# sarpaykent/GotenNet

Measured on AMD Instinct MI355X. Metric: molecules/sec (energy+force forward), rMD17 aspirin batch=128, 1/2/4/8 MI355X, higher is better.
Workload: dtype f32 (2xfp16-split MFMA with block exponents, fp32 accumulate); 1 GPU; rmd17_aspirin batch=128/GPU (N=2688 atoms, E=54368 edges incl. self-loops), n_atom_basis=256, n_interactions=6, lmax=2, n_rbf=32, heads=8, sep_dir/sep_tensor, energy+forces; global_batch=128, parallelism=dp1 (molecule shards, 1 all-reduce)

## Files before the change

gotennet_amd/_lib.py:

```python
from __future__ import annotations

import ctypes as C
import os

_PKG = os.path.dirname(os.path.abspath(__file__))
LIB_PATH = os.environ.get("GN_LIB_PATH") or os.path.join(_PKG, "libgotennet_hip.so")

GN_ERR_BAD_ARG = 10001
ABI_VERSION = 11
LMAX_SLICED = 0x100
LMAX_MEAN, LMAX_MAX = 0x200, 0x400

ACT_NONE = 11
WGRAD_F32, WGRAD_F16X2 = 0, 2
_P, _I, _F, _L, _D = C.c_void_p, C.c_int, C.c_float, C.c_long, C.c_double

class GemmDesc(C.Structure):
    _fields_ = [("A", _P), ("lda", _I), ("W", _P), ("bias", _P), ("C", _P), ("ldc", _I),
                ("M", _I), ("N", _I), ("K", _I), ("act_lo", _I), ("act_hi", _I),
                ("row_cnt", _I), ("row_gstride", _I), ("row_goff", _I),
                ("res", _P), ("gate", _P), ("gate_mode", _I), ("pre_out", _P),
                ("pro_mode", _I), ("pro_lo", _I), ("pro_hi", _I), ("a_pre", _P), ("ldp", _I),
                ("a_gate", _P), ("ldg", _I), ("A2", _P), ("A3", _P), ("a_seg", _I), ("act_kind", _I), ("lda2", _I)]


class WgradDesc(C.Structure):
    _fields_ = [("dY", _P), ("ldy", _I), ("y_off", _I), ("A", _P), ("lda", _I), ("a_off", _I),
                ("dW", _P), ("ldw", _I), ("db", _P), ("rows", _I), ("nout", _I), ("K", _I),
                ("row_cnt", _I), ("row_gstride", _I), ("row_goff", _I)]
# ... 26 lines not shown
    "gn_eqff_fused_backward": [_P, _P, _P, _P, _P, _P, _P, _P, _I, _I, _I, _P, _P, _I, _P],
    "gn_htr_edge": [_P, _P, _P, _P, _P, _I, _I, _I, _I, _P, _P, _P],
    "gn_eqff_context": [_P, _P, _F, _I, _I, _I, _P, _P],
    "gn_eqff_update": [_P, _P, _I, _I, _I, _P, _P, _P],
    "gn_gemm_ex": [_P, _I, _P, _P, _P, _I, _I, _I, _I, _I, _I, _I, _I, _I, _P, _P, _I, _P, _I, _I, _I, _P, _I, _P, _I, _I, _P],
    "gn_gemm_group": [_P, _I, _P],
    "gn_edge_vectors": [_P, _P, _P, _I, _P, _P, _P],
    "gn_gemm_split": [_P, _I, _P, _P, _P, _I, _I, _I, _I, _I, _I, _I, _I, _I, _P, _P, _I, _P, _I, _I, _I, _P, _I, _P, _I, _I, _P],
    "gn_split_bf16x3": [_P, _I, _I, _P, _P],
    "gn_split_bf16x3_size": [_I, _I],
    "gn_gemm_group_split": [_P, _I, _P],
    "gn_gemm_f16x2": [_P, _I, _P, _P, _P, _I, _I, _I, _I, _I, _I, _I, _I, _I, _P, _P, _I, _P, _I, _I, _I, _P, _I, _P, _I, _I, _P],
    "gn_split_f16x2": [_P, _I, _I, _P, _P],
    "gn_split_f16x2_size": [_I, _I],
    "gn_gemm_group_f16x2": [_P, _I, _P],
    "gn_htr_backward": [_P, _P, _P, _P, _P, _P, _P, _P, _P, _P, _P, _P, _I, _I, _I, _I, _P, _P, _P, _P, _I, _P],
    "gn_message_backward": [_P, _P, _I, _P, _I, _P, _P, _I, _P, _P, _P, _P, _P, _P, _P, _P, _P, _P, _P,
                            _P, _P, _P, _I, _P, _P, _P, _P, _P, _P, C.c_long, _I, _I, _I, _I, _I, _I, _I, _P],
    "gn_message_backward_dropout": [_P, _P, _I, _P, _I, _P, _P, _P, _I, _P, _P, _P, _P, _P, _P, _P, _P, _P, _P, _P,
                                    _P, _P, _P, _I, _P, _P, _P, _P, _P, _P, C.c_long, _I, _I, _I, _I, _I, _I, _I, _P],
    "gn_message_backward_groups": [_I, _I, _I, _I],
    "gn_eqff_backward_a": [_P, _P, _P, _P, _I, _I, _I, _P, _P, _P],
    "gn_eqff_backward_b": [_P, _P, _P, _P, _I, _I, _I, _P, _P, _P],
    "gn_edge_init_backward": [_P, _P, _P, _I, _P, _P, _P, _P, _I, _I, _P, _P, _P],
    "gn_node_init_backward": [_P, _P, _P, _I, _P, _P, _P, _P, _I, _I, _P, _P, _P],
    "gn_layernorm_silu_backward": [_P, _P, _P, _F, _P, _I, _I, _P, _I, _P],
    "gn_layernorm_backward": [_P, _P, _F, _P, _I, _I, _P, _P],
    "gn_tensor_norm_backward": [_P, _P, _P, _F, _I, _I, _I, _P, _P],
    "gn_gate": [_P, _I, _L, _P, _P],
    "gn_gate_backward": [_P, _P, _I, _L, _P, _P],
# ... 105 lines not shown
```

gotennet_amd/csrc/gn_gemm.hip:

```cpp
#include <climits>
#include <type_traits>
#include "gn_gemm.h"
#include "gn_tune.h"

namespace gn {

__device__ __forceinline__ float4 keep4(bool ok, const float4& v) {
    return make_float4(ok ? v.x : 0.f, ok ? v.y : 0.f, ok ? v.z : 0.f, ok ? v.w : 0.f);
}
__device__ __forceinline__ float amax4(const float4& v) { return fmaxf(fmaxf(fabsf(v.x), fabsf(v.y)), fmaxf(fabsf(v.z), fabsf(v.w))); }

template <int R>
__device__ __forceinline__ int block_exponent(const float4 (&v)[R]) {
    float m = 0.f;
#pragma unroll
    for (int i = 0; i < R; ++i) m = fmaxf(m, amax4(v[i]));
    int need = (int)((wave_umax_sgpr(__float_as_uint(m)) >> 23) & 0xffu) - 126 - 15;
    if (__builtin_expect(need > 112, 0)) {
        asm volatile("" ::: "memory");
        float mf = 0.f;
#pragma unroll
        for (int i = 0; i < R; ++i) {
            const float c[4] = {v[i].x, v[i].y, v[i].z, v[i].w};
#pragma unroll
            for (int t = 0; t < 4; ++t) mf = fmaxf(mf, fabsf(c[t]) <= 3.0e38f ? fabsf(c[t]) : 0.f);
        }
        need = (int)((wave_umax_sgpr(__float_as_uint(mf)) >> 23) & 0xffu) - 126 - 15;
    }
    return need < -120 ? -120 : need;
}
__device__ __forceinline__ void store_f16x2(_Float16* d, int apl, const float4& v, float scale) {
    f16x4 h, l;
    split4_f16(v, scale, h, l);
    *reinterpret_cast<f16x4*>(d) = h;
    *reinterpret_cast<f16x4*>(d + apl) = l;
}

template <int TM, int TN, int WM, int WN, bool PRO, int MODE, bool ASILU>
__device__ __forceinline__ void gemm_body(const GroupArgs ga) {
    static_assert(WM * WN == 4, "four waves per workgroup");
    constexpr bool SPLIT = MODE != 0;
    constexpr bool F16 = MODE == 2;
    constexpr int NP = F16 ? 2 : 3;
    constexpr int BM = 32 * TM * WM, BN = 32 * TN * WN;
    constexpr int RA = BM / 32, RB = BN / 32;
    constexpr int STAGE = (BM + BN) * PITCH;
    constexpr int CP = BN + 4;
    constexpr int APL = BM * SPLIT_PB;
    constexpr int STAGE_S = NP * APL;
    constexpr int MAIN_FLOATS = SPLIT ? (2 * STAGE_S) / 2 : 2 * STAGE;
    constexpr int LDS_FLOATS = (MAIN_FLOATS > BM * CP) ? MAIN_FLOATS : BM * CP;
    __shared__ __attribute__((aligned(16))) float smem[LDS_FLOATS + (F16 ? 2 : 0)];
    signed char* const exps = reinterpret_cast<signed char*>(smem + LDS_FLOATS);
    int e_run = -120;
    unsigned e_acc = 0x88888888u;
    int ewt = 0;

    int cum[GN_MAX_GROUP], shift[GN_MAX_GROUP];
    const int xcd = blockIdx.x & 7;
    if (ga.spread) {
        int run = 0, prev_end = 0;
#pragma unroll
        for (int gi = 0; gi < GN_MAX_GROUP; ++gi) {
            const int tg = gi < ga.n ? ga.tile_end[gi] - prev_end : 0;
            prev_end = gi < ga.n ? ga.tile_end[gi] : prev_end;
            const XcdCut c = xcd_cut(tg, xcd);
            shift[gi] = c.lo - run;
            run += c.cnt;
            cum[gi] = run;
        }
// ... 32 lines not shown
    const int wave = tid >> 6;
    const int wm = wave / WN, wn = wave % WN;
    const int c4 = tid & 7;
    const int sr = tid >> 3;
    const int stride = gridDim.x >> 3;

    int prow[RA];
    const float* brow[RB];
    bool aok[RA], bok[RB];
    bool a_full = false;
    auto set_tile = [&](int t_idx) {
        const int m0f = ((t_idx - g_begin) / tiles_n) * BM, n0f = ((t_idx - g_begin) % tiles_n) * BN;
        a_full = m0f + BM <= p.M && (p.K % BK) == 0;
#pragma unroll
        for (int i = 0; i < RA; ++i) {
            const int gm = m0f + sr + 32 * i;
            aok[i] = gm < p.M;
            prow[i] = phys_row(p, aok[i] ? gm : 0);
        }
        if constexpr (!SPLIT) {
#pragma unroll
            for (int i = 0; i < RB; ++i) {
                const int gn = n0f + sr + 32 * i;
                bok[i] = gn < p.N;
                brow[i] = p.W + (size_t)(bok[i] ? gn : 0) * p.K + 4 * c4;
            }
        }
    };

    f32x16 acc[TM][TN];

    float4 pa[RA], pb[RB];
    constexpr bool AHEAD = SPLIT && !PRO;
    float4 qa2[2][RA];
    bool kok2[2] = {true, true};
    auto fetchA = [&](int k0, float4 (&qa)[RA], bool& kflag) {
        const int kraw = k0 + 4 * c4;
        const bool kok = kraw < p.K;
// ... 5 lines not shown
            const bool s2 = k0c >= 2 * p.a_seg, s1 = k0c >= p.a_seg;
            Ab = s2 ? p.A3 : (s1 ? p.A2 : p.A);
            ka = kc - (s2 ? 2 * p.a_seg : (s1 ? p.a_seg : 0));
            ld = p.lda + ((p.lda2 - p.lda) & -(int)s1);
        }
#pragma unroll
        for (int i = 0; i < RA; ++i) qa[i] = ld4(Ab + (size_t)prow[i] * ld + ka);
        kflag = kok;
    };
    auto stash_f16 = [&](int sb, const float4 (&v)[RA]) {
        _Float16* d0 = reinterpret_cast<_Float16*>(smem) + sb * STAGE_S + sr * SPLIT_PB + 4 * c4;
        const int need = block_exponent(v);
        e_run = need > e_run ? need : e_run;
        const float scale = exp_scale(e_run);
#pragma unroll
        for (int i = 0; i < RA; ++i) store_f16x2(d0 + 32 * i * SPLIT_PB, APL, v[i], scale);
        if (lane == 0) exps[sb * 4 + wave] = (signed char)e_run;
    };
    auto stash_bf16 = [&](int sb, const float4 (&v)[RA]) {
        __bf16* d0 = reinterpret_cast<__bf16*>(smem) + sb * STAGE_S + sr * SPLIT_PB + 4 * c4;
#pragma unroll
        for (int i = 0; i < RA; ++i) {
            bf16x4 h, m, l;
            split4_trunc(v[i], h, m, l);
            __bf16* d = d0 + 32 * i * SPLIT_PB;
            *reinterpret_cast<bf16x4*>(d) = h;
            *reinterpret_cast<bf16x4*>(d + APL) = m;
            *reinterpret_cast<bf16x4*>(d + 2 * APL) = l;
        }
    };
    auto stashA = [&](int sb, const float4 (&qa)[RA], bool kflag) {
        if constexpr (F16) {
            if (a_full) {
                stash_f16(sb, qa);
                return;
            }
        }
        float4 v[RA];
#pragma unroll
        for (int i = 0; i < RA; ++i) v[i] = keep4(aok[i] && kflag, qa[i]);
// ... 29 lines not shown
        if constexpr (!SPLIT) {
#pragma unroll
            for (int i = 0; i < RB; ++i) qb[i] = (bok[i] && kok) ? ld4(brow[i] + k0) : zero4();
        }
    };
    auto stash = [&](int sb, const float4 (&qa)[RA], const float4 (&qb)[RB]) {
        if constexpr (AHEAD) {
            stashA(sb, qa2[0], kok2[0]);
        } else if constexpr (F16) {
            stash_f16(sb, qa);
        } else if constexpr (SPLIT) {
            stash_bf16(sb, qa);
        } else {
            float* buf = smem + sb * STAGE;
#pragma unroll
            for (int i = 0; i < RA; ++i) st4(&buf[(sr + 32 * i) * PITCH + 4 * c4], qa[i]);
#pragma unroll
            for (int i = 0; i < RB; ++i) st4(&buf[(BM + sr + 32 * i) * PITCH + 4 * c4], qb[i]);
        }
    };
    const uint4* wfrag = reinterpret_cast<const uint4*>(p.W);
    int ks2 = 0;
    size_t nt_off[TN];
    auto set_btile = [&](int n0b) {
        wfrag = reinterpret_cast<const uint4*>(p.W) + (F16 ? 16 : 0);
        if constexpr (F16) ewt = __builtin_amdgcn_readfirstlane(*reinterpret_cast<const int*>(p.W));
        ks2 = 2 * ((p.K + BK - 1) / BK);
        const int nt_last = (p.N + 31) / 32 - 1;
#pragma unroll
        for (int j = 0; j < TN; ++j) {
            int nt = n0b / 32 + wn * TN + j;
            nt = nt < nt_last ? nt : nt_last;
            nt_off[j] = (size_t)nt * ks2 * (NP * 64) + lane;
        }
    };
    auto load_b = [&](int g, uint4 (&q)[TN][NP]) {
#pragma unroll
        for (int j = 0; j < TN; ++j)
#pragma unroll
            for (int s_ = 0; s_ < NP; ++s_) q[j][s_] = wfrag[nt_off[j] + (size_t)(g * NP + s_) * 64];
    };
    auto rescale = [&](int sb) {
        const unsigned en = (unsigned)__builtin_amdgcn_readfirstlane(*reinterpret_cast<const int*>(exps + sb * 4));
        if (__builtin_expect(en != e_acc, 0)) {
            rescale_rows(&acc[0][0], TM * TN, e_acc, en);
            e_acc = en;
        }
    };

    auto kstep = [&](const __bf16* Ap, int ks, const uint4 (&bw)[TN][NP]) {
        if constexpr (F16) {
            f16x8 a[TM][2];
#pragma unroll
            for (int i = 0; i < TM; ++i)
#pragma unroll
                for (int s_ = 0; s_ < 2; ++s_)
                    a[i][s_] = *reinterpret_cast<const f16x8*>(Ap + s_ * APL + i * 32 * SPLIT_PB + ks * 16);
#pragma unroll
            for (int t = 0; t < 3; ++t)
#pragma unroll
                for (int i = 0; i < TM; ++i)
// ... 9 lines not shown
                for (int s_ = 0; s_ < 3; ++s_)
                    a[i][s_] = *reinterpret_cast<const bf16x8*>(Ap + s_ * APL + i * 32 * SPLIT_PB + ks * 16);
            constexpr int TA[6] = {2, 0, 1, 1, 0, 0};
            constexpr int TB[6] = {0, 2, 1, 0, 1, 0};
#pragma unroll
            for (int t = 0; t < 6; ++t)
#pragma unroll
                for (int i = 0; i < TM; ++i)
#pragma unroll
                    for (int j = 0; j < TN; ++j)
                        acc[i][j] = __builtin_amdgcn_mfma_f32_32x32x16_bf16(
                            a[i][TA[t]], __builtin_bit_cast(bf16x8, bw[j][TB[t]]), acc[i][j], 0, 0, 0);
        }
    };

    auto loop_planes_ahead = [&](int nk, uint4 (&bq)[2][TN][NP]) {
        const __bf16* const Abase = reinterpret_cast<const __bf16*>(smem) + (wm * 32 * TM + (lane & 31)) * SPLIT_PB + (lane >> 5) * 8;
        auto slab = [&](int kt, auto SET, auto LAST) {
            constexpr int set = decltype(SET)::value;
            constexpr bool last = decltype(LAST)::value;
            const __bf16* Ap = Abase + set * STAGE_S;
            load_b(2 * kt + 1, bq[1]);
            if constexpr (!last) fetchA((kt + 2) * BK, qa2[set], kok2[set]);
            __builtin_amdgcn_sched_barrier(0);
            if constexpr (F16) rescale(set);
            kstep(Ap, 0, bq[0]);
            __builtin_amdgcn_sched_barrier(0);
            if constexpr (!last) load_b(2 * kt + 2, bq[0]);
            kstep(Ap, 1, bq[1]);
            __builtin_amdgcn_sched_barrier(0);
            if constexpr (!last) stashA(set ^ 1, qa2[set ^ 1], kok2[set ^ 1]);
            __syncthreads();
        };
        using T0 = std::integral_constant<int, 0>; using T1 = std::integral_constant<int, 1>;
        using No = std::false_type; using Yes = std::true_type;
        fetchA(BK, qa2[1], kok2[1]);
        int kt = 0;
        for (; kt + 2 < nk; kt += 2) {
            slab(kt, T0{}, No{});
            slab(kt + 1, T1{}, No{});
        }
        if (nk - kt == 2) {
            slab(kt, T0{}, No{});
            slab(kt + 1, T1{}, Yes{});
        } else {
            slab(kt, T0{}, Yes{});
        }
    };

    int idx = blockIdx.x >> 3;
    if (idx >= tile_stop) return;
    select(idx);
    set_tile(idx);
    fetch(0, pa, pb);
    for (;;) {
        const int nk = (p.K + BK - 1) / BK;
        const int m0 = ((idx - g_begin) / tiles_n) * BM;
        const int n0 = ((idx - g_begin) % tiles_n) * BN;
#pragma unroll
        for (int i = 0; i < TM; ++i)
#pragma unroll
            for (int j = 0; j < TN; ++j)
#pragma unroll
                for (int r = 0; r < 16; ++r) acc[i][j][r] = 0.f;
        if constexpr (F16) {
            e_run = -120;
            e_acc = 0x88888888u;
        }
        stash(0, pa, pb);
        uint4 bq[2][TN][NP];
        if constexpr (SPLIT) {
            set_btile(n0);
            load_b(0, bq[0]);
        }
        __syncthreads();
        if constexpr (AHEAD) loop_planes_ahead(nk, bq);
        else if constexpr (SPLIT) {
            const __bf16* const Abase = reinterpret_cast<const __bf16*>(smem) + (wm * 32 * TM + (lane & 31)) * SPLIT_PB + (lane >> 5) * 8;
            if (nk > 1) fetch(BK, pa, pb);
            for (int kt = 0; kt < nk; ++kt) {
                const __bf16* Ap = Abase + (kt & 1) * STAGE_S;
                load_b(2 * kt + 1, bq[1]);
                if constexpr (F16) rescale(kt & 1);
                kstep(Ap, 0, bq[0]);
                if (kt + 1 < nk) load_b(2 * kt + 2, bq[0]);
                kstep(Ap, 1, bq[1]);
                if (kt + 1 < nk) stash((kt + 1) & 1, pa, pb);
                __syncthreads();
                if (kt + 2 < nk) fetch((kt + 2) * BK, pa, pb);
            }
        }
// ... 40 lines not shown
        const bool same = has_next && next < g_end;
        if (same) {
            set_tile(next);
            fetch(0, pa, pb);
        }

        {
#pragma unroll
        for (int i = 0; i < TM; ++i)
#pragma unroll
            for (int j = 0; j < TN; ++j)
#pragma unroll
                for (int r = 0; r < 16; ++r) {
                    const int row = wm * 32 * TM + i * 32 + (r & 3) + 8 * (r >> 2) + 4 * (lane >> 5);
                    float v = acc[i][j][r];
                    if constexpr (F16) v = ldexpf(v, (int)(signed char)(e_acc >> (8 * (r >> 2))) + ewt);
                    smem[row * CP + wn * 32 * TN + j * 32 + (lane & 31)] = v;
                }
        __syncthreads();
        {
            constexpr int C4 = BN / 4;
            const int cc = (tid % C4) * 4, gn = n0 + cc;
            if (gn < p.N) {
                const float4 bias4 = p.bias ? ld4(p.bias + gn) : zero4();
                const bool act = gn >= p.act_lo && gn < p.act_hi;
                const int kind = ASILU ? (int)GN_ACT_SILU : p.act_kind;
                if (p.res || p.gate) {
                    constexpr int ITS = (BM * C4) / 256, UN = ITS < 4 ? ITS : 4;
                    for (int it0 = 0; it0 < ITS; it0 += UN) {
                        size_t off[UN];
                        bool ok[UN];
                        float4 rv[UN], gv[UN];
#pragma unroll
                        for (int u = 0; u < UN; ++u) {
                            const int gm = m0 + (it0 + u) * (256 / C4) + tid / C4;
                            ok[u] = gm < p.M;
                            off[u] = (size_t)phys_row(p, ok[u] ? gm : 0) * p.ldc + gn;
                            rv[u] = (ok[u] && p.res) ? ld4(p.res + off[u]) : zero4();
                            gv[u] = (ok[u] && p.gate) ? ld4(p.gate + off[u]) : zero4();
                        }
#pragma unroll
                        for (int u = 0; u < UN; ++u) {
                            if (!ok[u]) continue;
                            const int row = (it0 + u) * (256 / C4) + tid / C4;
                            float4 v = ld4(&smem[row * CP + cc]) + bias4;
                            if (p.pre_out) st4(p.pre_out + off[u], v);
                            if (act) v = act4(v, ASILU ? (int)GN_ACT_SILU : p.act_kind);
                            if (p.gate) v = v * (p.gate_mode ? dact4(gv[u], ASILU ? (int)GN_ACT_SILU : p.act_kind) : gv[u]);
                            if (p.res) v = rv[u] + v;
                            st4(p.C + off[u], v);
                        }
                    }
                } else {
#pragma unroll 4
                    for (int it = 0; it < (BM * C4) / 256; ++it) {
                        const int row = it * (256 / C4) + tid / C4;
                        const int gm = m0 + row;
                        if (gm >= p.M) continue;
                        const float4 x = ld4(&smem[row * CP + cc]);
                        const size_t off = (size_t)phys_row(p, gm) * p.ldc + gn;
                        epi_store<true>(x, bias4, off, p.C, p.pre_out, act, kind, nullptr, 0, zero4(), nullptr, zero4(), gn, p.nt_store);
                    }
                }
            }
        }
        __syncthreads();
        }
        if (!has_next) break;
        if (!same) {
            select(next);
            set_tile(next);
// ... 2 lines not shown
        idx = next;
    }
}

template <int TM, int TN, int WM, int WN, bool PRO, bool ASILU>
__global__ __launch_bounds__(256) void gemm_f32_mfma(const GroupArgs ga) {
    gemm_body<TM, TN, WM, WN, PRO, 0, ASILU>(ga);
}

template <int TM, int TN, int WM, int WN, bool PRO, bool ASILU>
__global__ __launch_bounds__(256, GN_SPLIT_MINW) void gemm_bf16x3_mfma(const GroupArgs ga) {
    gemm_body<TM, TN, WM, WN, PRO, 1, ASILU>(ga);
}

template <int TM, int TN, int WM, int WN, bool PRO, bool ASILU>
__global__ __launch_bounds__(256, GN_SPLIT_MINW) void gemm_f16x2_mfma(const GroupArgs ga) {
    gemm_body<TM, TN, WM, WN, PRO, 2, ASILU>(ga);
}

}

namespace {
using gn::GemmArgs;
using SlabKernel = void (*)(const gn::GroupArgs);

enum Tile { TILE_BIG, TILE_MID, TILE_WIDE, TILE_SMALL, TILE_COUNT };
struct TileShape {
    int TM, TN, WM, WN;
    constexpr int BM() const { return 32 * TM * WM; }
    constexpr int BN() const { return 32 * TN * WN; }
};
constexpr TileShape SLAB_TILES[3][TILE_COUNT] = {
    {{2, 2, 2, 2}, {0, 0, 0, 0}, {0, 0, 0, 0}, {1, 1, 2, 2}},
    {{4, 1, 1, 4}, {0, 0, 0, 0}, {0, 0, 0, 0}, {1, 1, 2, 2}},
    {{4, 1, 1, 4}, {2, 1, 1, 4}, {1, 1, 1, 4}, {1, 1, 2, 2}},
};

template <int MODE, int T, bool PRO, bool ASILU>
SlabKernel slab_kernel() {
    constexpr TileShape s = SLAB_TILES[MODE][T];
    if constexpr (s.TM == 0) return nullptr;
    else if constexpr (MODE == 0) return gn::gemm_f32_mfma<s.TM, s.TN, s.WM, s.WN, PRO, ASILU>;
    else if constexpr (MODE == 1) return gn::gemm_bf16x3_mfma<s.TM, s.TN, s.WM, s.WN, PRO, ASILU>;
    else return gn::gemm_f16x2_mfma<s.TM, s.TN, s.WM, s.WN, PRO, ASILU>;
}
template <int MODE, int T>
SlabKernel slab_kernel(bool pro, bool silu) {
    return pro ? (silu ? slab_kernel<MODE, T, true, true>() : slab_kernel<MODE, T, true, false>())
               : (silu ? slab_kernel<MODE, T, false, true>() : slab_kernel<MODE, T, false, false>());
}
template <int MODE>
SlabKernel slab_kernel(Tile t, bool pro, bool silu) {
    switch (t) {
    case TILE_BIG: return slab_kernel<MODE, TILE_BIG>(pro, silu);
    case TILE_MID: return slab_kernel<MODE, TILE_MID>(pro, silu);
    case TILE_WIDE: return slab_kernel<MODE, TILE_WIDE>(pro, silu);
    default: return slab_kernel<MODE, TILE_SMALL>(pro, silu);
    }
}

struct TilePlan { Tile tile; long cap; };
TilePlan tile_plan(const GemmArgs* g, int n, int split) {
    long big = 0, rows_all = 0;
    bool wide = GN_F16_SMALL_WIDE && split == 2, gated = false;
    for (int i = 0; i < n; ++i) {
        big += (long)((g[i].M + 127) / 128) * ((g[i].N + 127) / 128);
        wide = wide && g[i].N >= 128;
        rows_all += g[i].M;
        gated = gated || (g[i].gate != nullptr && g[i].res != nullptr);
    }
    if (big >= (long)GN_GEMM_BIG_MIN) return {TILE_BIG, GN_GEMM_BIG_CAP};
    if (wide && gated && GN_F16_MID_ROWS > 0 && rows_all >= (long)GN_F16_MID_ROWS) return {TILE_MID, GN_F16_MID_CAP};
    if (wide) return {TILE_WIDE, GN_F16_SMALL_CAP};
    return {TILE_SMALL, 1024};
}

int slab_launch(const GemmArgs* g, int n, hipStream_t st, int split) {
    const TilePlan plan = tile_plan(g, n, split);
    const TileShape shape = SLAB_TILES[split][plan.tile];
    gn::GroupArgs ga;
    const long tiles = gn::fill_group(ga, ga.tile_end, g, n, shape.BM(), shape.BN());
    if (tiles == 0) return GN_OK;
    ga.spread = 0;
    bool pro = false, silu = true;
    for (int i = 0; i < n; ++i) {
        const long t0 = ga.tile_end[0], ti = ga.tile_end[i] - (i ? ga.tile_end[i - 1] : 0);
        ga.spread |= (g[i].K != g[0].K) || ti * 4 < t0 || t0 * 4 < ti;
        pro = pro || g[i].pro_mode != 0 || g[i].a_gate != nullptr;
        silu = silu && g[i].act_kind == GN_ACT_SILU;
    }
    long grid = 8L * ((tiles + 7) / 8);
    if (grid > plan.cap) grid = plan.cap;
    const SlabKernel k = split == 2 ? slab_kernel<2>(plan.tile, pro, silu)
                       : split == 1 ? slab_kernel<1>(plan.tile, pro, silu) : slab_kernel<0>(plan.tile, pro, silu);
    hipLaunchKernelGGL(k, dim3((unsigned)grid), dim3(256), 0, st, ga);
    GN_LAUNCH_CHECK();
    return GN_OK;
}

bool act_kind_ok(int k) { return k >= 0 && k < GN_ACT_COUNT; }

bool desc_ok(const gn_gemm_desc& q) {
    if (q.M < 0 || q.N <= 0 || q.K <= 0 || (q.K & 3) || (q.lda & 3) || (q.N & 3) || (q.ldc & 3) || (q.act_lo & 3) ||
        (q.act_hi & 3) || q.row_cnt <= 0)
        return false;
    if (q.gate != nullptr && q.res == nullptr && q.gate_mode == 0) return false;
    if (q.pro_mode < 0 || q.pro_mode > 2 || (q.pro_mode == 2 && (!q.a_pre || (q.ldp & 3))) || (q.a_gate && (q.ldg & 3)) ||
        (q.pro_mode && ((q.pro_lo & 3) || (q.pro_hi & 3))))
        return false;
    if (q.a_seg < 0 || (q.a_seg && ((q.a_seg % gn::BK) || q.pro_mode || q.a_gate || q.K > 3 * q.a_seg ||
// ... 9 lines not shown
    p.a_pre = q.a_pre; p.a_gate = q.a_gate;
    p.lda = q.lda; p.ldc = q.ldc; p.ldp = q.ldp; p.ldg = q.ldg;
    p.M = q.M; p.N = q.N; p.K = q.K;
    p.act_lo = q.act_lo; p.act_hi = q.act_hi;
    p.pro_mode = q.pro_mode; p.pro_lo = q.pro_lo; p.pro_hi = q.pro_hi;
    p.row_cnt = q.row_cnt; p.row_gstride = q.row_gstride; p.row_goff = q.row_goff;
    p.gate_mode = q.gate_mode;
    p.A2 = q.A2; p.A3 = q.A3; p.a_seg = q.a_seg;
    p.act_kind = q.act_kind;
    p.lda2 = q.lda2 ? q.lda2 : q.lda;
    const int nt_lo = GN_GEMM_NT_LO >= 0 ? GN_GEMM_NT_LO : q.K;
    p.nt_store = (double)q.M * q.N * 4.0 >= (double)GN_GEMM_NT_MB * 1048576.0 ? (q.N > nt_lo ? nt_lo : 0) : INT_MAX;
    return p;
}

int gemm_launch(const GemmArgs* g, int n, hipStream_t st, int split) {
    if (split == 2) {
        int r = gn_gemm_panel_launch(g, n, st);
        if (r == 0) r = gn_gemm_colpipe_launch(g, n, st);
        if (r != 0) return r > 0 ? GN_OK : -r;
    }
    return slab_launch(g, n, st, split);
}

int gemm_group_impl(const gn_gemm_desc* d, int n, void* stream, int split) {
    if (n < 0 || n > gn::GN_MAX_GROUP || (n > 0 && !d)) return GN_ERR_BAD_ARG;
    GemmArgs g[gn::GN_MAX_GROUP];
    int m = 0;
    for (int i = 0; i < n; ++i) {
        if (!desc_ok(d[i])) return GN_ERR_BAD_ARG;
        if (d[i].M != 0) g[m++] = make_args(d[i]);
    }
    if (m == 0) return GN_OK;
    return gemm_launch(g, m, (hipStream_t)stream, split);
}

int gemm_single(const float* A, int lda, const void* W, const float* bias, float* C, int ldc, int Mrows, int Nout, int K,
                int act_lo, int act_hi, int row_cnt, int row_gstride, int row_goff, const float* res, const float* gate,
                int gate_mode, float* pre_out, int pro_mode, int pro_lo, int pro_hi, const float* a_pre, int ldp,
                const float* a_gate, int ldg, int act_kind, void* stream, int split) {
    if (!act_kind_ok(act_kind) || (split && !W)) return GN_ERR_BAD_ARG;
    gn_gemm_desc d{};
    d.A = A; d.lda = lda; d.W = static_cast<const float*>(W); d.bias = bias; d.C = C; d.ldc = ldc;
    d.M = Mrows; d.N = Nout; d.K = K; d.act_lo = act_lo; d.act_hi = act_hi;
    d.row_cnt = row_cnt; d.row_gstride = row_gstride; d.row_goff = row_goff;
    d.res = res; d.gate = gate; d.gate_mode = gate_mode; d.pre_out = pre_out;
    d.pro_mode = pro_mode; d.pro_lo = pro_lo; d.pro_hi = pro_hi; d.a_pre = a_pre; d.ldp = ldp; d.a_gate = a_gate; d.ldg = ldg;
    d.act_kind = act_kind;
    return gemm_group_impl(&d, 1, stream, split);
}
}

extern "C" int gn_gemm_group(const gn_gemm_desc* d, int n, void* stream) { return gemm_group_impl(d, n, stream, 0); }
extern "C" int gn_gemm_group_split(const gn_gemm_desc* d, int n, void* stream) { return gemm_group_impl(d, n, stream, 1); }
extern "C" int gn_gemm_group_f16x2(const gn_gemm_desc* d, int n, void* stream) { return gemm_group_impl(d, n, stream, 2); }

extern "C" int gn_gemm_ex(const float* A, int lda, const float* W, const float* bias, float* C, int ldc, int Mrows, int Nout,
        int K, int act_lo, int act_hi, int row_cnt, int row_gstride, int row_goff, const float* res, const float* gate,
        int gate_mode, float* pre_out, int pro_mode, int pro_lo, int pro_hi, const float* a_pre, int ldp,
        const float* a_gate, int ldg, int act_kind, void* stream) {
    return gemm_single(A, lda, W, bias, C, ldc, Mrows, Nout, K, act_lo, act_hi, row_cnt, row_gstride, row_goff, res, gate,
                       gate_mode, pre_out, pro_mode, pro_lo, pro_hi, a_pre, ldp, a_gate, ldg, act_kind, stream, 0);
}

extern "C" int gn_gemm_split(const float* A, int lda, const unsigned short* W3, const float* bias, float* C, int ldc, int Mrows, int Nout,
        int K, int act_lo, int act_hi, int row_cnt, int row_gstride, int row_goff, const float* res, const float* gate,
        int gate_mode, float* pre_out, int pro_mode, int pro_lo, int pro_hi, const float* a_pre, int ldp,
        const float* a_gate, int ldg, int act_kind, void* stream) {
    return gemm_single(A, lda, W3, bias, C, ldc, Mrows, Nout, K, act_lo, act_hi, row_cnt, row_gstride, row_goff, res, gate,
                       gate_mode, pre_out, pro_mode, pro_lo, pro_hi, a_pre, ldp, a_gate, ldg, act_kind, stream, 1);
// ... 17 lines not shown
```

gotennet_amd/csrc/gn_tune.h:

```cpp
#pragma once

#define GN_WPE_ATTR(n) __attribute__((amdgpu_waves_per_eu(n, n)))

#ifndef GN_W_K6
#define GN_W_K6 3
#endif
#ifndef GN_W_K6_G
#define GN_W_K6_G 3
#endif
#ifndef GN_W_MSG_TGT
#define GN_W_MSG_TGT 0
#endif
#ifndef GN_W_MSG_SRC
#define GN_W_MSG_SRC 2
#endif
#ifndef GN_W_HTR_TGT
#define GN_W_HTR_TGT 0
#endif
#ifndef GN_W_HTR_SRC
#define GN_W_HTR_SRC 0
#endif
#ifndef GN_W_HTR_SRC_G
#define GN_W_HTR_SRC_G 0
#endif
// ... 48 lines not shown
#ifndef GN_GEMM_PANEL_MAX
#define GN_GEMM_PANEL_MAX 2048
#endif
#ifndef GN_F16_SMALL_WIDE
#define GN_F16_SMALL_WIDE 1
#endif
#ifndef GN_F16_MID_ROWS
#define GN_F16_MID_ROWS 30000
#endif
#ifndef GN_F16_MID_CAP
#define GN_F16_MID_CAP 768
#endif
#ifndef GN_F16_SMALL_CAP
#define GN_F16_SMALL_CAP 1024
#endif
#ifndef GN_HTR_CLOSED
#define GN_HTR_CLOSED 1
#endif
#ifndef GN_HTR_CLOSED_ALL
#define GN_HTR_CLOSED_ALL 4
#endif
#ifndef GN_ATTN_WAVE
#define GN_ATTN_WAVE 1
#endif

#define GN_TUNE_CAT_(a, b) a##b
#define GN_TUNE_CAT(a, b) GN_TUNE_CAT_(a, b)
#define GN_WPE_SEL_0
#define GN_WPE_SEL_1 GN_WPE_ATTR(1)
#define GN_WPE_SEL_2 GN_WPE_ATTR(2)
// ... 7 lines not shown
```

gotennet_amd/engine.py:

```python
from __future__ import annotations

import dataclasses
import os
from dataclasses import dataclass, field
from typing import Any, List, Optional

import torch

from . import _lib
from ._lib import call, ptr


@dataclass
class LayerWeights:
    Wn1: Optional[torch.Tensor] = None; bn1: Optional[torch.Tensor] = None
    Ws2: Optional[torch.Tensor] = None; bs2: Optional[torch.Tensor] = None
    Wv2: Optional[torch.Tensor] = None; bv2: Optional[torch.Tensor] = None
    We: Optional[torch.Tensor] = None; be: Optional[torch.Tensor] = None
    Wvu: Optional[torch.Tensor] = None
    Wm0: Optional[torch.Tensor] = None; bm0: Optional[torch.Tensor] = None
    Wm1: Optional[torch.Tensor] = None; bm1: Optional[torch.Tensor] = None
    Wt: Optional[torch.Tensor] = None; bt: Optional[torch.Tensor] = None
    Wvq: Optional[torch.Tensor] = None
    Wvk: List[torch.Tensor] = field(default_factory=list)
# ... 167 lines not shown

def gemm(A, lda, W, bias, C, ldc, rows, nout, K, act=(0, 0), rowmap=(1, 1, 0), res=None, gate=None,
         a_off=0, c_off=0, pre_out=None, pro=(0, 0, 0), a_pre=None, ldp=0, p_off=0, a_gate=None, ldg=0,
         dgate=None, g_off=0, kind=None, mode=None):
    mode = resolve_mode(mode)
    name = "gn_gemm_ex"
    if mode in _PLANE_MODES:
        name, W = _PLANE_MODES[mode][0], split_weight(W, mode)
    call(name, A.data_ptr() + 4 * a_off, lda, ptr(W), ptr(bias), C.data_ptr() + 4 * c_off, ldc,
         rows, nout, K, act[0], act[1], rowmap[0], rowmap[1], rowmap[2], ptr(res),
         (dgate.data_ptr() + 4 * g_off) if dgate is not None else ptr(gate), 1 if dgate is not None else 0, ptr(pre_out),
         pro[0], pro[1], pro[2], (a_pre.data_ptr() + 4 * p_off) if a_pre is not None else None, ldp,
         ptr(a_gate), ldg, 0 if kind is None else kind, _stream())


def gemm_group(problems, mode=None, kind=None):
    mode = resolve_mode(mode)
    kind = 0 if kind is None else kind
    problems = [q for q in problems if q is not None]
    split = mode in _PLANE_MODES
    for i0 in range(0, len(problems), 4):
        chunk = problems[i0:i0 + 4]
        arr = (_lib.GemmDesc * len(chunk))()
        for d, q in zip(arr, chunk):
            g = q.get
            act, rowmap, pro = g("act", (0, 0)), g("rowmap", (1, 1, 0)), g("pro", (0, 0, 0))
            dgate = g("dgate")
            d.A = q["A"].data_ptr() + 4 * g("a_off", 0); d.lda = q["lda"]
            d.W = ptr(split_weight(q["W"], mode) if split else q["W"]); d.bias = ptr(g("bias"))
            d.C = q["C"].data_ptr() + 4 * g("c_off", 0); d.ldc = q["ldc"]
            d.M, d.N, d.K = q["rows"], q["nout"], q["K"]
            d.act_lo, d.act_hi = act
            d.row_cnt, d.row_gstride, d.row_goff = rowmap
            d.res = ptr(g("res"))
            d.gate = (dgate.data_ptr() + 4 * g("g_off", 0)) if dgate is not None else ptr(g("gate"))
            d.gate_mode = 1 if dgate is not None else 0
            d.pre_out = ptr(g("pre_out"))
            d.pro_mode, d.pro_lo, d.pro_hi = pro
            a_pre = g("a_pre")
            d.a_pre = (a_pre.data_ptr() + 4 * g("p_off", 0)) if a_pre is not None else None
            d.ldp = g("ldp", 0)
            d.a_gate = ptr(g("a_gate")); d.ldg = g("ldg", 0)
            d.A2, d.A3, d.a_seg = ptr(g("A2")), ptr(g("A3")), g("a_seg", 0)
            d.act_kind = g("kind", kind)
            d.lda2 = g("lda2", 0)
        call(_PLANE_MODES[mode][1] if split else "gn_gemm_group", arr, len(chunk), _stream())


class _Call:
    __slots__ = ("mode", "act", "cfg", "g", "st", "N", "E", "F", "D", "Fe", "lde", "blocks", "cols", "key")

    def __init__(self, cfg: "Config", g: Optional["Graph"] = None, explicit_blocks: bool = False,
                 key: Optional[torch.Tensor] = None):
        self.key = key
        self.mode, self.act, self.cfg, self.g, self.st = resolve_mode(cfg.gemm_mode), cfg.act, cfg, g, _stream()
        self.F, self.D, self.Fe, self.lde = cfg.F, cfg.D, cfg.Fe, (1 + cfg.M) * cfg.F
        n = cfg.lmax if cfg.sep_dir else 1
        self.cols = ((self.lde, cfg.M * cfg.F), ((2 + n) * cfg.F, (1 + n) * cfg.F))
        self.N, self.E = (g.N, g.E) if g is not None else (None, None)
        self.blocks = cfg.degree_blocks(g.N, explicit_blocks) if g is not None else None
# ... 834 lines not shown
```

include/gotennet_hip.h:

```cpp
#ifndef GOTENNET_HIP_H
#define GOTENNET_HIP_H

#include <stdint.h>

#ifdef __cplusplus
extern "C" {
#endif

#define GN_OK 0
#define GN_ERR_BAD_ARG 10001
#define GN_ABI_VERSION 11
#define GN_LMAX_SLICED 0x100
#define GN_LMAX_MEAN 0x200
#define GN_LMAX_MAX 0x400

enum {
    GN_ACT_SILU = 0, GN_ACT_SSP = 1, GN_ACT_RELU = 2, GN_ACT_TANH = 3, GN_ACT_SIGMOID = 4, GN_ACT_ELU = 5,
    GN_ACT_SELU = 6, GN_ACT_MISH = 7, GN_ACT_GELU = 8, GN_ACT_SOFTPLUS = 9, GN_ACT_LEAKY = 10,
    GN_ACT_NONE = 11 , GN_ACT_COUNT = 12
};

int gn_abi_version(const char** arch_out);


// ... 75 lines not shown
                  int row_cnt, int row_gstride, int row_goff,
                  const float* res, const float* gate, int gate_mode, float* pre_out,
                  int pro_mode, int pro_lo, int pro_hi, const float* a_pre, int ldp,
                  const float* a_gate, int ldg, int act_kind, void* stream);
int gn_gemm_group_split(const gn_gemm_desc* problems, int n, void* stream);

long gn_split_f16x2_size(int N, int K);
int gn_split_f16x2(const float* w , int N, int K, unsigned short* out, void* stream);
int gn_gemm_f16x2(const float* A, int lda, const unsigned short* W2, const float* bias, float* C, int ldc,
                  int Mrows, int Nout, int K, int act_lo, int act_hi,
                  int row_cnt, int row_gstride, int row_goff,
                  const float* res, const float* gate, int gate_mode, float* pre_out,
                  int pro_mode, int pro_lo, int pro_hi, const float* a_pre, int ldp,
                  const float* a_gate, int ldg, int act_kind, void* stream);
int gn_gemm_group_f16x2(const gn_gemm_desc* problems, int n, void* stream);

int gn_attn_softmax(const float* q, const float* k, int ldqk, const float* t_attn, int ldt,
                    const int* rowptr, const int* src, const int* outdeg,
                    int N, int F, int H, float* a, int act , void* stream);

int gn_attn_softmax_dropout(const float* q, const float* k, int ldqk, const float* t_attn, int ldt,
                            const int* rowptr, const int* src, const int* outdeg,
                            int N, int F, int H, float* a_soft, float* a, const long long* key, int layer, double p,
                            int act, void* stream);
int gn_attn_dropout_mask(const long long* key, int layer, double p, long E, int H, float* m_out, void* stream);

int gn_message_aggregate(const float* x, const float* v, int ldxv, const float* t_filter, int ldt,
                         const float* a, const float* rl, const float* cut,
                         const int* rowptr, const int* src,
                         const float* h_in, const float* X_in, float* h_out, float* X_out,
// ... 218 lines not shown
```

Measured before the change: 22760 molecules/s.

## Add 8-wave 128x256 f16x2 GEMM tile with phase-staggered A prefetch

After: 23070 molecules/s, median of 6. 1.01x the previous value.

```diff
diff --git a/gotennet_amd/_lib.py b/gotennet_amd/_lib.py
--- a/gotennet_amd/_lib.py
+++ b/gotennet_amd/_lib.py
@@ -13,6 +13,7 @@
 
 ACT_NONE = 11
 WGRAD_F32, WGRAD_F16X2 = 0, 2
+GEMM_FORM_BIG, GEMM_FORM_BIG8 = 1, 2
 _P, _I, _F, _L, _D = C.c_void_p, C.c_int, C.c_float, C.c_long, C.c_double
 
 class GemmDesc(C.Structure):
@@ -69,6 +70,7 @@
     "gn_split_f16x2": [_P, _I, _I, _P, _P],
     "gn_split_f16x2_size": [_I, _I],
     "gn_gemm_group_f16x2": [_P, _I, _P],
+    "gn_gemm_group_f16x2_form": [_P, _I, _I, _P],
     "gn_htr_backward": [_P, _P, _P, _P, _P, _P, _P, _P, _P, _P, _P, _P, _I, _I, _I, _I, _P, _P, _P, _P, _I, _P],
     "gn_message_backward": [_P, _P, _I, _P, _I, _P, _P, _I, _P, _P, _P, _P, _P, _P, _P, _P, _P, _P, _P,
                             _P, _P, _P, _I, _P, _P, _P, _P, _P, _P, C.c_long, _I, _I, _I, _I, _I, _I, _I, _P],
diff --git a/gotennet_amd/csrc/gn_gemm.hip b/gotennet_amd/csrc/gn_gemm.hip
--- a/gotennet_amd/csrc/gn_gemm.hip
+++ b/gotennet_amd/csrc/gn_gemm.hip
@@ -38,22 +38,27 @@
 
 template <int TM, int TN, int WM, int WN, bool PRO, int MODE, bool ASILU>
 __device__ __forceinline__ void gemm_body(const GroupArgs ga) {
-    static_assert(WM * WN == 4, "four waves per workgroup");
+    constexpr int NW = WM * WN, NT = 64 * NW;
+    static_assert(NW == 4 || (NW == 8 && MODE == 2 && WM == 1), "four waves per workgroup, or 1 x 8 in the f16x2 arithmetic");
     constexpr bool SPLIT = MODE != 0;
     constexpr bool F16 = MODE == 2;
     constexpr int NP = F16 ? 2 : 3;
     constexpr int BM = 32 * TM * WM, BN = 32 * TN * WN;
-    constexpr int RA = BM / 32, RB = BN / 32;
+    constexpr int SRS = 8 * NW;
+    constexpr int RA = BM / SRS, RB = BN / SRS;
+    constexpr int EG = NW / 4;
     constexpr int STAGE = (BM + BN) * PITCH;
     constexpr int CP = BN + 4;
     constexpr int APL = BM * SPLIT_PB;
     constexpr int STAGE_S = NP * APL;
     constexpr int MAIN_FLOATS = SPLIT ? (2 * STAGE_S) / 2 : 2 * STAGE;
     constexpr int LDS_FLOATS = (MAIN_FLOATS > BM * CP) ? MAIN_FLOATS : BM * CP;
-    __shared__ __attribute__((aligned(16))) float smem[LDS_FLOATS + (F16 ? 2 : 0)];
+    __shared__ __attribute__((aligned(16))) float smem[LDS_FLOATS + (F16 ? 2 * EG : 0)];
     signed char* const exps = reinterpret_cast<signed char*>(smem + LDS_FLOATS);
     int e_run = -120;
-    unsigned e_acc = 0x88888888u;
+    unsigned e_acc[EG];
+#pragma unroll
+    for (int g = 0; g < EG; ++g) e_acc[g] = 0x88888888u;
     int ewt = 0;
 
     int cum[GN_MAX_GROUP], shift[GN_MAX_GROUP];
@@ -116,14 +121,14 @@
         a_full = m0f + BM <= p.M && (p.K % BK) == 0;
 #pragma unroll
         for (int i = 0; i < RA; ++i) {
-            const int gm = m0f + sr + 32 * i;
+            const int gm = m0f + sr + SRS * i;
             aok[i] = gm < p.M;
             prow[i] = phys_row(p, aok[i] ? gm : 0);
         }
         if constexpr (!SPLIT) {
 #pragma unroll
             for (int i = 0; i < RB; ++i) {
-                const int gn = n0f + sr + 32 * i;
+                const int gn = n0f + sr + SRS * i;
                 bok[i] = gn < p.N;
                 brow[i] = p.W + (size_t)(bok[i] ? gn : 0) * p.K + 4 * c4;
             }
@@ -159,8 +164,8 @@
         e_run = need > e_run ? need : e_run;
         const float scale = exp_scale(e_run);
 #pragma unroll
-        for (int i = 0; i < RA; ++i) store_f16x2(d0 + 32 * i * SPLIT_PB, APL, v[i], scale);
-        if (lane == 0) exps[sb * 4 + wave] = (signed char)e_run;
+        for (int i = 0; i < RA; ++i) store_f16x2(d0 + SRS * i * SPLIT_PB, APL, v[i], scale);
+        if (lane == 0) exps[sb * NW + wave] = (signed char)e_run;
     };
     auto stash_bf16 = [&](int sb, const float4 (&v)[RA]) {
         __bf16* d0 = reinterpret_cast<__bf16*>(smem) + sb * STAGE_S + sr * SPLIT_PB + 4 * c4;
@@ -168,7 +173,7 @@
         for (int i = 0; i < RA; ++i) {
             bf16x4 h, m, l;
             split4_trunc(v[i], h, m, l);
-            __bf16* d = d0 + 32 * i * SPLIT_PB;
+            __bf16* d = d0 + SRS * i * SPLIT_PB;
             *reinterpret_cast<bf16x4*>(d) = h;
             *reinterpret_cast<bf16x4*>(d + APL) = m;
             *reinterpret_cast<bf16x4*>(d + 2 * APL) = l;
@@ -228,9 +233,9 @@
         } else {
             float* buf = smem + sb * STAGE;
 #pragma unroll
-            for (int i = 0; i < RA; ++i) st4(&buf[(sr + 32 * i) * PITCH + 4 * c4], qa[i]);
-#pragma unroll
-            for (int i = 0; i < RB; ++i) st4(&buf[(BM + sr + 32 * i) * PITCH + 4 * c4], qb[i]);
+            for (int i = 0; i < RA; ++i) st4(&buf[(sr + SRS * i) * PITCH + 4 * c4], qa[i]);
+#pragma unroll
+            for (int i = 0; i < RB; ++i) st4(&buf[(BM + sr + SRS * i) * PITCH + 4 * c4], qb[i]);
         }
     };
     const uint4* wfrag = reinterpret_cast<const uint4*>(p.W);
@@ -255,10 +260,26 @@
             for (int s_ = 0; s_ < NP; ++s_) q[j][s_] = wfrag[nt_off[j] + (size_t)(g * NP + s_) * 64];
     };
     auto rescale = [&](int sb) {
-        const unsigned en = (unsigned)__builtin_amdgcn_readfirstlane(*reinterpret_cast<const int*>(exps + sb * 4));
-        if (__builtin_expect(en != e_acc, 0)) {
-            rescale_rows(&acc[0][0], TM * TN, e_acc, en);
-            e_acc = en;
+        if constexpr (EG == 1) {
+            const unsigned en = (unsigned)__builtin_amdgcn_readfirstlane(*reinterpret_cast<const int*>(exps + sb * 4));
+            if (__builtin_expect(en != e_acc[0], 0)) {
+                rescale_rows(&acc[0][0], TM * TN, e_acc[0], en);
+                e_acc[0] = en;
+            }
+        } else {
+            unsigned en[EG];
+            bool same = true;
+#pragma unroll
+            for (int g = 0; g < EG; ++g) {
+                en[g] = (unsigned)__builtin_amdgcn_readfirstlane(*reinterpret_cast<const int*>(exps + sb * NW + 4 * g));
+                same = same && en[g] == e_acc[g];
+            }
+            if (__builtin_expect(!same, 0)) {
+#pragma unroll
+                for (int i = 0; i < TM; ++i) rescale_rows(&acc[i][0], TN, e_acc[i % EG], en[i % EG]);
+#pragma unroll
+                for (int g = 0; g < EG; ++g) e_acc[g] = en[g];
+            }
         }
     };
 
@@ -298,14 +319,21 @@
         }
     };
 
-    auto loop_planes_ahead = [&](int nk, uint4 (&bq)[2][TN][NP]) {
+    auto loop_planes_ahead = [&](int nk, uint4 (&bq)[2][TN][NP], auto EARLY) {
+        constexpr bool early = decltype(EARLY)::value;
         const __bf16* const Abase = reinterpret_cast<const __bf16*>(smem) + (wm * 32 * TM + (lane & 31)) * SPLIT_PB + (lane >> 5) * 8;
         auto slab = [&](int kt, auto SET, auto LAST) {
             constexpr int set = decltype(SET)::value;
             constexpr bool last = decltype(LAST)::value;
             const __bf16* Ap = Abase + set * STAGE_S;
             load_b(2 * kt + 1, bq[1]);
-            if constexpr (!last) fetchA((kt + 2) * BK, qa2[set], kok2[set]);
+            if constexpr (!early) {
+                if constexpr (!last) fetchA((kt + 2) * BK, qa2[set], kok2[set]);
+            } else if constexpr (!last) {
+                stashA(set ^ 1, qa2[set ^ 1], kok2[set ^ 1]);
+                __builtin_amdgcn_sched_barrier(0);
+                fetchA((kt + 3) * BK, qa2[set ^ 1], kok2[set ^ 1]);
+            }
             __builtin_amdgcn_sched_barrier(0);
             if constexpr (F16) rescale(set);
             kstep(Ap, 0, bq[0]);
@@ -313,12 +341,13 @@
             if constexpr (!last) load_b(2 * kt + 2, bq[0]);
             kstep(Ap, 1, bq[1]);
             __builtin_amdgcn_sched_barrier(0);
-            if constexpr (!last) stashA(set ^ 1, qa2[set ^ 1], kok2[set ^ 1]);
+            if constexpr (!last && !early) stashA(set ^ 1, qa2[set ^ 1], kok2[set ^ 1]);
             __syncthreads();
         };
         using T0 = std::integral_constant<int, 0>; using T1 = std::integral_constant<int, 1>;
         using No = std::false_type; using Yes = std::true_type;
         fetchA(BK, qa2[1], kok2[1]);
+        if constexpr (early) fetchA(2 * BK, qa2[0], kok2[0]);
         int kt = 0;
         for (; kt + 2 < nk; kt += 2) {
             slab(kt, T0{}, No{});
@@ -349,7 +378,8 @@
                 for (int r = 0; r < 16; ++r) acc[i][j][r] = 0.f;
         if constexpr (F16) {
             e_run = -120;
-            e_acc = 0x88888888u;
+#pragma unroll
+            for (int g = 0; g < EG; ++g) e_acc[g] = 0x88888888u;
         }
         stash(0, pa, pb);
         uint4 bq[2][TN][NP];
@@ -358,7 +388,10 @@
             load_b(0, bq[0]);
         }
         __syncthreads();
-        if constexpr (AHEAD) loop_planes_ahead(nk, bq);
+        if constexpr (AHEAD && NW == 8 && GN_F16_BIG8_PHASED) {
+            if (GN_F16_BIG8_PHASED == 2 ? (__builtin_amdgcn_readfirstlane(wave) & 1) : (__builtin_amdgcn_readfirstlane(wave) >= 4)) loop_planes_ahead(nk, bq, std::true_type{});
+            else loop_planes_ahead(nk, bq, std::false_type{});
+        } else if constexpr (AHEAD) loop_planes_ahead(nk, bq, std::false_type{});
         else if constexpr (SPLIT) {
             const __bf16* const Abase = reinterpret_cast<const __bf16*>(smem) + (wm * 32 * TM + (lane & 31)) * SPLIT_PB + (lane >> 5) * 8;
             if (nk > 1) fetch(BK, pa, pb);
@@ -429,7 +462,7 @@
                 for (int r = 0; r < 16; ++r) {
                     const int row = wm * 32 * TM + i * 32 + (r & 3) + 8 * (r >> 2) + 4 * (lane >> 5);
                     float v = acc[i][j][r];
-                    if constexpr (F16) v = ldexpf(v, (int)(signed char)(e_acc >> (8 * (r >> 2))) + ewt);
+                    if constexpr (F16) v = ldexpf(v, (int)(signed char)(e_acc[i % EG] >> (8 * (r >> 2))) + ewt);
                     smem[row * CP + wn * 32 * TN + j * 32 + (lane & 31)] = v;
                 }
         __syncthreads();
@@ -441,14 +474,14 @@
                 const bool act = gn >= p.act_lo && gn < p.act_hi;
                 const int kind = ASILU ? (int)GN_ACT_SILU : p.act_kind;
                 if (p.res || p.gate) {
-                    constexpr int ITS = (BM * C4) / 256, UN = ITS < 4 ? ITS : 4;
+                    constexpr int ITS = (BM * C4) / NT, UN = ITS < 4 ? ITS : 4;
                     for (int it0 = 0; it0 < ITS; it0 += UN) {
                         size_t off[UN];
                         bool ok[UN];
                         float4 rv[UN], gv[UN];
 #pragma unroll
                         for (int u = 0; u < UN; ++u) {
-                            const int gm = m0 + (it0 + u) * (256 / C4) + tid / C4;
+                            const int gm = m0 + (it0 + u) * (NT / C4) + tid / C4;
                             ok[u] = gm < p.M;
                             off[u] = (size_t)phys_row(p, ok[u] ? gm : 0) * p.ldc + gn;
                             rv[u] = (ok[u] && p.res) ? ld4(p.res + off[u]) : zero4();
@@ -457,7 +490,7 @@
 #pragma unroll
                         for (int u = 0; u < UN; ++u) {
                             if (!ok[u]) continue;
-                            const int row = (it0 + u) * (256 / C4) + tid / C4;
+                            const int row = (it0 + u) * (NT / C4) + tid / C4;
                             float4 v = ld4(&smem[row * CP + cc]) + bias4;
                             if (p.pre_out) st4(p.pre_out + off[u], v);
                             if (act) v = act4(v, ASILU ? (int)GN_ACT_SILU : p.act_kind);
@@ -468,8 +501,8 @@
                     }
                 } else {
 #pragma unroll 4
-                    for (int it = 0; it < (BM * C4) / 256; ++it) {
-                        const int row = it * (256 / C4) + tid / C4;
+                    for (int it = 0; it < (BM * C4) / NT; ++it) {
+                        const int row = it * (NT / C4) + tid / C4;
                         const int gm = m0 + row;
                         if (gm >= p.M) continue;
                         const float4 x = ld4(&smem[row * CP + cc]);
@@ -502,7 +535,7 @@
 }
 
 template <int TM, int TN, int WM, int WN, bool PRO, bool ASILU>
-__global__ __launch_bounds__(256, GN_SPLIT_MINW) void gemm_f16x2_mfma(const GroupArgs ga) {
+__global__ __launch_bounds__(64 * WM * WN, GN_SPLIT_MINW) void gemm_f16x2_mfma(const GroupArgs ga) {
     gemm_body<TM, TN, WM, WN, PRO, 2, ASILU>(ga);
 }
 
@@ -512,22 +545,22 @@
 using gn::GemmArgs;
 using SlabKernel = void (*)(const gn::GroupArgs);
 
-enum Tile { TILE_BIG, TILE_MID, TILE_WIDE, TILE_SMALL, TILE_COUNT };
+enum Tile { TILE_BIG, TILE_MID, TILE_WIDE, TILE_SMALL, TILE_BIG8, TILE_COUNT };
 struct TileShape {
     int TM, TN, WM, WN;
     constexpr int BM() const { return 32 * TM * WM; }
     constexpr int BN() const { return 32 * TN * WN; }
 };
 constexpr TileShape SLAB_TILES[3][TILE_COUNT] = {
-    {{2, 2, 2, 2}, {0, 0, 0, 0}, {0, 0, 0, 0}, {1, 1, 2, 2}},
-    {{4, 1, 1, 4}, {0, 0, 0, 0}, {0, 0, 0, 0}, {1, 1, 2, 2}},
-    {{4, 1, 1, 4}, {2, 1, 1, 4}, {1, 1, 1, 4}, {1, 1, 2, 2}},
+    {{2, 2, 2, 2}, {0, 0, 0, 0}, {0, 0, 0, 0}, {1, 1, 2, 2}, {0, 0, 0, 0}},
+    {{4, 1, 1, 4}, {0, 0, 0, 0}, {0, 0, 0, 0}, {1, 1, 2, 2}, {0, 0, 0, 0}},
+    {{4, 1, 1, 4}, {2, 1, 1, 4}, {1, 1, 1, 4}, {1, 1, 2, 2}, {4, 1, 1, 8}},
 };
 
 template <int MODE, int T, bool PRO, bool ASILU>
 SlabKernel slab_kernel() {
     constexpr TileShape s = SLAB_TILES[MODE][T];
-    if constexpr (s.TM == 0) return nullptr;
+    if constexpr (s.TM == 0 || (T == TILE_BIG8 && PRO)) return nullptr;
     else if constexpr (MODE == 0) return gn::gemm_f32_mfma<s.TM, s.TN, s.WM, s.WN, PRO, ASILU>;
     else if constexpr (MODE == 1) return gn::gemm_bf16x3_mfma<s.TM, s.TN, s.WM, s.WN, PRO, ASILU>;
     else return gn::gemm_f16x2_mfma<s.TM, s.TN, s.WM, s.WN, PRO, ASILU>;
@@ -543,45 +576,54 @@
     case TILE_BIG: return slab_kernel<MODE, TILE_BIG>(pro, silu);
     case TILE_MID: return slab_kernel<MODE, TILE_MID>(pro, silu);
     case TILE_WIDE: return slab_kernel<MODE, TILE_WIDE>(pro, silu);
+    case TILE_BIG8: return slab_kernel<MODE, TILE_BIG8>(pro, silu);
     default: return slab_kernel<MODE, TILE_SMALL>(pro, silu);
     }
 }
 
 struct TilePlan { Tile tile; long cap; };
-TilePlan tile_plan(const GemmArgs* g, int n, int split) {
+TilePlan tile_plan(const GemmArgs* g, int n, int split, bool pro, int form) {
+    if (form == GN_GEMM_FORM_BIG) return {TILE_BIG, GN_GEMM_BIG_CAP};
+    if (form == GN_GEMM_FORM_BIG8) return {TILE_BIG8, GN_F16_BIG8_CAP};
     long big = 0, rows_all = 0;
     bool wide = GN_F16_SMALL_WIDE && split == 2, gated = false;
+    bool big8 = GN_F16_BIG8_MIN_K > 0 && split == 2 && !pro && g[0].K >= GN_F16_BIG8_MIN_K && g[0].N > 128;
     for (int i = 0; i < n; ++i) {
         big += (long)((g[i].M + 127) / 128) * ((g[i].N + 127) / 128);
         wide = wide && g[i].N >= 128;
+        big8 = big8 && g[i].N <= 256;
         rows_all += g[i].M;
         gated = gated || (g[i].gate != nullptr && g[i].res != nullptr);
     }
+    if (big8 && big >= (long)GN_GEMM_BIG_MIN) return {TILE_BIG8, GN_F16_BIG8_CAP};
     if (big >= (long)GN_GEMM_BIG_MIN) return {TILE_BIG, GN_GEMM_BIG_CAP};
     if (wide && gated && GN_F16_MID_ROWS > 0 && rows_all >= (long)GN_F16_MID_ROWS) return {TILE_MID, GN_F16_MID_CAP};
     if (wide) return {TILE_WIDE, GN_F16_SMALL_CAP};
     return {TILE_SMALL, 1024};
 }
 
-int slab_launch(const GemmArgs* g, int n, hipStream_t st, int split) {
-    const TilePlan plan = tile_plan(g, n, split);
+int slab_launch(const GemmArgs* g, int n, hipStream_t st, int split, int form = 0) {
+    bool pro = false, silu = true;
+    for (int i = 0; i < n; ++i) {
+        pro = pro || g[i].pro_mode != 0 || g[i].a_gate != nullptr;
+        silu = silu && g[i].act_kind == GN_ACT_SILU;
+    }
+    if (form != 0 && (split != 2 || (form == GN_GEMM_FORM_BIG8 && pro))) return GN_ERR_BAD_ARG;
+    const TilePlan plan = tile_plan(g, n, split, pro, form);
     const TileShape shape = SLAB_TILES[split][plan.tile];
     gn::GroupArgs ga;
     const long tiles = gn::fill_group(ga, ga.tile_end, g, n, shape.BM(), shape.BN());
     if (tiles == 0) return GN_OK;
     ga.spread = 0;
-    bool pro = false, silu = true;
     for (int i = 0; i < n; ++i) {
         const long t0 = ga.tile_end[0], ti = ga.tile_end[i] - (i ? ga.tile_end[i - 1] : 0);
         ga.spread |= (g[i].K != g[0].K) || ti * 4 < t0 || t0 * 4 < ti;
-        pro = pro || g[i].pro_mode != 0 || g[i].a_gate != nullptr;
-        silu = silu && g[i].act_kind == GN_ACT_SILU;
     }
     long grid = 8L * ((tiles + 7) / 8);
     if (grid > plan.cap) grid = plan.cap;
     const SlabKernel k = split == 2 ? slab_kernel<2>(plan.tile, pro, silu)
                        : split == 1 ? slab_kernel<1>(plan.tile, pro, silu) : slab_kernel<0>(plan.tile, pro, silu);
-    hipLaunchKernelGGL(k, dim3((unsigned)grid), dim3(256), 0, st, ga);
+    hipLaunchKernelGGL(k, dim3((unsigned)grid), dim3(64 * shape.WM * shape.WN), 0, st, ga);
     GN_LAUNCH_CHECK();
     return GN_OK;
 }
@@ -621,7 +663,8 @@
     return p;
 }
 
-int gemm_launch(const GemmArgs* g, int n, hipStream_t st, int split) {
+int gemm_launch(const GemmArgs* g, int n, hipStream_t st, int split, int form) {
+    if (form != 0) return slab_launch(g, n, st, split, form);
     if (split == 2) {
         int r = gn_gemm_panel_launch(g, n, st);
         if (r == 0) r = gn_gemm_colpipe_launch(g, n, st);
@@ -630,7 +673,7 @@
     return slab_launch(g, n, st, split);
 }
 
-int gemm_group_impl(const gn_gemm_desc* d, int n, void* stream, int split) {
+int gemm_group_impl(const gn_gemm_desc* d, int n, void* stream, int split, int form = 0) {
     if (n < 0 || n > gn::GN_MAX_GROUP || (n > 0 && !d)) return GN_ERR_BAD_ARG;
     GemmArgs g[gn::GN_MAX_GROUP];
     int m = 0;
@@ -639,7 +682,7 @@
         if (d[i].M != 0) g[m++] = make_args(d[i]);
     }
     if (m == 0) return GN_OK;
-    return gemm_launch(g, m, (hipStream_t)stream, split);
+    return gemm_launch(g, m, (hipStream_t)stream, split, form);
 }
 
 int gemm_single(const float* A, int lda, const void* W, const float* bias, float* C, int ldc, int Mrows, int Nout, int K,
@@ -661,6 +704,10 @@
 extern "C" int gn_gemm_group(const gn_gemm_desc* d, int n, void* stream) { return gemm_group_impl(d, n, stream, 0); }
 extern "C" int gn_gemm_group_split(const gn_gemm_desc* d, int n, void* stream) { return gemm_group_impl(d, n, stream, 1); }
 extern "C" int gn_gemm_group_f16x2(const gn_gemm_desc* d, int n, void* stream) { return gemm_group_impl(d, n, stream, 2); }
+extern "C" int gn_gemm_group_f16x2_form(const gn_gemm_desc* d, int n, int form, void* stream) {
+    if (form != GN_GEMM_FORM_BIG && form != GN_GEMM_FORM_BIG8) return GN_ERR_BAD_ARG;
+    return gemm_group_impl(d, n, stream, 2, form);
+}
 
 extern "C" int gn_gemm_ex(const float* A, int lda, const float* W, const float* bias, float* C, int ldc, int Mrows, int Nout,
         int K, int act_lo, int act_hi, int row_cnt, int row_gstride, int row_goff, const float* res, const float* gate,
diff --git a/gotennet_amd/csrc/gn_tune.h b/gotennet_amd/csrc/gn_tune.h
--- a/gotennet_amd/csrc/gn_tune.h
+++ b/gotennet_amd/csrc/gn_tune.h
@@ -86,6 +86,15 @@
 #ifndef GN_F16_SMALL_CAP
 #define GN_F16_SMALL_CAP 1024
 #endif
+#ifndef GN_F16_BIG8_MIN_K
+#define GN_F16_BIG8_MIN_K 1024
+#endif
+#ifndef GN_F16_BIG8_CAP
+#define GN_F16_BIG8_CAP 256
+#endif
+#ifndef GN_F16_BIG8_PHASED
+#define GN_F16_BIG8_PHASED 1
+#endif
 #ifndef GN_HTR_CLOSED
 #define GN_HTR_CLOSED 1
 #endif
diff --git a/gotennet_amd/engine.py b/gotennet_amd/engine.py
--- a/gotennet_amd/engine.py
+++ b/gotennet_amd/engine.py
@@ -205,8 +205,10 @@
          ptr(a_gate), ldg, 0 if kind is None else kind, _stream())
 
 
-def gemm_group(problems, mode=None, kind=None):
+def gemm_group(problems, mode=None, kind=None, form=0):
     mode = resolve_mode(mode)
+    if form and mode != "f16x2":
+        raise ValueError("a named slab-kernel form is an f16x2 launch")
     kind = 0 if kind is None else kind
     problems = [q for q in problems if q is not None]
     split = mode in _PLANE_MODES
@@ -235,6 +237,9 @@
             d.A2, d.A3, d.a_seg = ptr(g("A2")), ptr(g("A3")), g("a_seg", 0)
             d.act_kind = g("kind", kind)
             d.lda2 = g("lda2", 0)
+        if form:
+            call("gn_gemm_group_f16x2_form", arr, len(chunk), form, _stream())
+            continue
         call(_PLANE_MODES[mode][1] if split else "gn_gemm_group", arr, len(chunk), _stream())
 
 
diff --git a/include/gotennet_hip.h b/include/gotennet_hip.h
--- a/include/gotennet_hip.h
+++ b/include/gotennet_hip.h
@@ -113,6 +113,9 @@
                   int pro_mode, int pro_lo, int pro_hi, const float* a_pre, int ldp,
                   const float* a_gate, int ldg, int act_kind, void* stream);
 int gn_gemm_group_f16x2(const gn_gemm_desc* problems, int n, void* stream);
+#define GN_GEMM_FORM_BIG 1
+#define GN_GEMM_FORM_BIG8 2
+int gn_gemm_group_f16x2_form(const gn_gemm_desc* problems, int n, int form, void* stream);
 
 int gn_attn_softmax(const float* q, const float* k, int ldqk, const float* t_attn, int ldt,
                     const int* rowptr, const int* src, const int* outdeg,
```
